# Jianxff/svo_pro_universal

Measured on AMD Instinct MI355X. Metric: aligned patches/sec + ms/frame, EuRoC 640x480 mono, 1/2/4/8 MI355X, higher is better.
Workload: dtype f64

## Files before the change

### svo_pro_universal_amd/csrc/context.hip

```cpp
#include <cmath>
#include <cstdarg>
#include <algorithm>
#include <cstring>

#include "svoh_internal.h"
#include "svoh_math.h"

namespace svoh {

static thread_local std::string g_global_err = "no error";

int set_error(svoh_ctx* ctx, int code, const char* fmt, ...)
{
  char buf[1024];
  va_list ap;
  va_start(ap, fmt);
  vsnprintf(buf, sizeof buf, fmt, ap);
  va_end(ap);
  if (ctx) ctx->err = buf; else g_global_err = buf;
  return code;
}

void set_global_error(const char* msg) { g_global_err = msg; }

// ... 351 lines not shown

__global__ __launch_bounds__(64) void camera_maths_wide_kernel(const svoh_camera cam, int n, const double* xyz, double* px, double* J, double* f_back)
{
  const int i = blockIdx.x * 64 + threadIdx.x;
  if (i >= n) return;
  const CamModelWide cm = load_camera_wide(cam);
  const Vec3 p = { xyz[3 * i], xyz[3 * i + 1], xyz[3 * i + 2] };
  double u, v;
  project3(cm, p, u, v);
  px[2 * i] = u; px[2 * i + 1] = v;
  if (J) {
    double Jl[6];
    project3_jacobian(cm, p, Jl);
    for (int k = 0; k < 6; ++k) J[6 * i + k] = Jl[k];
  }
  const Vec3 f = back_project3(cm, u, v);
  f_back[3 * i] = f.x; f_back[3 * i + 1] = f.y; f_back[3 * i + 2] = f.z;
}

void load_knobs_from_env(SvohKnobs& k)
{
  auto get = [](const char* name) { const char* e = getenv(name); return e ? atoi(e) : kKnobUnset; };
  k.klt_block = get("SVOH_KLT_BLOCK");
  k.matcher_g8 = get("SVOH_MATCHER_G8");
  k.seed_binning = get("SVOH_SEED_BINNING");
  k.pose_threads = get("SVOH_POSE_THREADS");
  k.align_cluster = get("SVOH_ALIGN_CLUSTER");
#ifdef SVOH_TEST_HOOKS
  k.align_cluster_test_absent = get("SVOH_ALIGN_CLUSTER_TEST_ABSENT");
#endif
  k.align_threads = get("SVOH_ALIGN_THREADS");
  k.align_rows = get("SVOH_ALIGN_ROWS");
  k.align_latency_build = get("SVOH_ALIGN_LATENCY_BUILD");
  k.align_lds = get("SVOH_ALIGN_LDS");
  k.align_wg_per_cu = get("SVOH_ALIGN_WG_PER_CU");
  k.kernel_timing = get("SVOH_KERNEL_TIMING");
  k.copy_kernel = get("SVOH_COPY_KERNEL");
}

static int build_pyramid_levels(svoh_ctx* ctx, hipStream_t stream, const std::shared_ptr<Slab>& slab, uint8_t* base, size_t fbytes, const size_t* offs, const int* ws,
                                const int* hs, int n_images, int width, int height, int n_levels, int rounding, svoh_frame_t* out_frames);

extern "C" {

int svoh_abi_version(void) { return SVOH_ABI_VERSION; }

int svoh_set_kernel_timing(svoh_ctx* ctx, int enabled)
try {
  if (!ctx) return set_error(nullptr, SVOH_ERR_INVALID_ARGUMENT, "ctx is NULL");
  ctx->knobs.kernel_timing = enabled ? 1 : 0;
  return SVOH_OK;
} SVOH_ABI_CATCH(ctx)

int svoh_set_copy_policy(svoh_ctx* ctx, int policy)
try {
  if (!ctx) return set_error(nullptr, SVOH_ERR_INVALID_ARGUMENT, "ctx is NULL");
  SVOH_REQUIRE(ctx, policy >= 0 && policy <= 2, "copy policy: 0 the runtime's copies, 1 copy kernels for 16 KB .. 1 MB, 2 copy kernels always");
  ctx->knobs.copy_kernel = policy;
  return SVOH_OK;
} SVOH_ABI_CATCH(ctx)

int svoh_reload_knobs(svoh_ctx* ctx)
try {
  if (!ctx) return set_error(nullptr, SVOH_ERR_INVALID_ARGUMENT, "ctx is NULL");
  const int timing = ctx->knobs.kernel_timing, copy_policy = ctx->knobs.copy_kernel;
  load_knobs_from_env(ctx->knobs);
// ... 465 lines not shown
```

### svo_pro_universal_amd/csrc/sparse_align.hip

```cpp
#include <atomic>
#include <cstdlib>
#include <cstring>

#include <type_traits>

#include "svoh_internal.h"
#include "svoh_device_utils.h"
#include "svoh_math.h"

#define SVOH_ALIGN_DRAIN(ctx) do { SVOH_HIP_TRY(ctx, hipStreamSynchronize((ctx)->stream)); (ctx)->align_launches_since_drain = 0; } while (0)

namespace svoh {

struct DevCamDesc {
  DevImage ref[SVOH_MAX_LEVELS];
  DevImage cur[SVOH_MAX_LEVELS];
  svoh_camera cam;
  svoh_se3 ref_T_imu_cam, ref_T_cam_imu, cur_T_cam_imu;
  double ref_pos[3];
  const double* px;
  const double* f;
  const double* pos_world;
  const uint8_t* flags;
  int32_t n_features;
// ... 6 lines not shown
  double alpha_init, beta_init;
  svoh_align_prior prior;
};

struct AlignKernelArgs {
  const DevProblemDesc* problems;
  const DevCamDesc* cams;
  svoh_align_result* results;
  double* wpk;
  int64_t slots;
  uint8_t* wsel;
  uint8_t* wvis;
  svoh_align_options opt;
  int32_t lds_img_bytes;
  int32_t rig_build;
  int32_t latency_build;
  int32_t lds_two_per_cu;
  int32_t ws_lds_bytes;
  int32_t eval_level;
  double* eval_out;
  long long* stamps;
  int32_t n_problems;
  int32_t* queue;
  int32_t one_each;
  const svoh_align_gn_state* ext_state;
  int32_t raw_sums;
  int32_t cluster;
  double* xchg;
  unsigned int* bar;
#ifdef SVOH_TEST_HOOKS
  int32_t cluster_test_absent;
#endif
};

constexpr int kXchgStride = 64;

#ifndef SVOH_ROW_UNROLL_GONLY
#define SVOH_ROW_UNROLL_GONLY 4
#endif
#ifndef SVOH_PIN_MOMENTS
#define SVOH_PIN_MOMENTS 1
#endif
#ifndef SVOH_ALIGN_WAVE_STEP
#define SVOH_ALIGN_WAVE_STEP 1
#endif
#ifndef SVOH_STEP_PRIO
#define SVOH_STEP_PRIO 1
#endif
#ifndef SVOH_ROW_UNROLL
#define SVOH_ROW_UNROLL (PH == 8 ? 4 : (D == 8 ? 1 : 2))
#endif

#ifdef SVOH_PHASE_STAMPS
#define SVOH_STAMP_DECL long long st_t0 = 0, st_acc[8] = {0, 0, 0, 0, 0, 0, 0, 0}; const long long st_begin = (long long)__builtin_amdgcn_s_memtime();
#define SVOH_STAMP_START() do { st_t0 = (long long)__builtin_amdgcn_s_memtime(); } while (0)
#define SVOH_STAMP_ADD(k) do { long long st_n = (long long)__builtin_amdgcn_s_memtime(); st_acc[k] += st_n - st_t0; st_t0 = st_n; } while (0)
#define SVOH_STAMP_COUNT(k) do { st_acc[k] += 1; } while (0)
#define SVOH_STAMP_FLUSH() do { if (threadIdx.x == 0) { st_acc[7] = (long long)__builtin_amdgcn_s_memtime() - st_begin; for (int k_ = 0; k_ < 8; ++k_) a.stamps[pbi * 20 + k_] = st_acc[k_]; for (int k_ = 0; k_ < 4; ++k_) a.stamps[pbi * 20 + 8 + k_] = g_state.dbg[k_]; for (int k_ = 0; k_ < 8; ++k_) a.stamps[pbi * 20 + 12 + k_] = g_state.dbg2[k_]; } } while (0)
#define SVOH_SERIAL_STAMP(k) do { long long st_n = (long long)__builtin_amdgcn_s_memtime(); s.dbg[k] += st_n - st_s0; st_s0 = st_n; } while (0)
#define SVOH_PASS_STAMP_BEGIN() long long ps_t0 = 0; if (threadIdx.x == 0) { __builtin_amdgcn_s_waitcnt(0); ps_t0 = (long long)__builtin_amdgcn_s_memtime(); }
#define SVOH_PASS_STAMP(k) do { if (threadIdx.x == 0) { __builtin_amdgcn_s_waitcnt(0); long long ps_n = (long long)__builtin_amdgcn_s_memtime(); g_state.dbg2[k] += ps_n - ps_t0; ps_t0 = ps_n; } } while (0)
#define SVOH_OUTER_STAMP_BEGIN() long long os_t0 = 0; if (threadIdx.x == 0) { __builtin_amdgcn_s_waitcnt(0); os_t0 = (long long)__builtin_amdgcn_s_memtime(); }
#define SVOH_OUTER_STAMP(k) do { if (threadIdx.x == 0) { __builtin_amdgcn_s_waitcnt(0); long long os_n = (long long)__builtin_amdgcn_s_memtime(); g_state.dbg2[k] += os_n - os_t0; os_t0 = os_n; } } while (0)
#else
#define SVOH_PASS_STAMP_BEGIN()
#define SVOH_PASS_STAMP(k) do {} while (0)
// ... 1066 lines not shown
    for (int j = 0; j < 8; ++j) { const double v = fabs(xg[j]); if (v > x_norm) x_norm = v; }
    if (x_norm < opt.eps) level_done = 1;
    __builtin_amdgcn_wave_barrier();
    if (lane == 0) {
      s.Told = T; s.alpha_old = alpha; s.beta_old = beta;
      s.T = Tn; s.alpha = an; s.beta = bn;
      if (level_done) s.level_done = 1;
    }
    T = Tn; alpha = an; beta = bn;
  }
  SVOH_WAVE_STAMP(2);
  {
    const int c = lane < n_cams ? lane : 0;
    const Rigid Tcr = mul(mul(s.cam_cur_T_cam_imu[c], T), s.cam_ref_T_imu_cam[c]);
    if (lane < n_cams) s.Tcr[c] = Tcr;
    if (lane == 0) { s.alpha_f = (float)alpha; s.beta_f = (float)beta; }
  }
  SVOH_WAVE_STAMP(3);
}

#ifndef SVOH_ALIGN_STAGED
#define SVOH_ALIGN_STAGED 1
#endif
#ifndef SVOH_ALIGN_REUSE_HESSIAN
#define SVOH_ALIGN_REUSE_HESSIAN 1
#endif
#ifndef SVOH_ALIGN_MIN_WAVES_256
#define SVOH_ALIGN_MIN_WAVES_256 2
#endif
#ifndef SVOH_ALIGN_ROWS_DEFAULT
#define SVOH_ALIGN_ROWS_DEFAULT(fit) (fit)
#endif

template <int P, int NT, bool ILLUM, bool CLUSTER = false, bool ROBUST = false, int LPP = 1, bool LAT = false, bool RIG = false>
__global__ __launch_bounds__(NT, (NT == 256 ? (LAT ? 1 : SVOH_ALIGN_MIN_WAVES_256) : 2))
void sparse_align_kernel(const AlignKernelArgs a)
{
  static_assert(!LAT || (NT == 256 && !CLUSTER && LPP == 1), "latency build: the 256-thread lane-per-patch geometry");
  static_assert(!RIG || (!CLUSTER && LPP == 1 && (LAT || NT == 512)), "rig build: the two lane-per-patch geometries of small launches");
  static_assert(LPP == 1 || (!CLUSTER && NT == 512 && LPP <= P), "rows geometry: 512 threads, no cluster mode");
  static_assert(NT == 256 || NT == 512, "workgroups of 256 or 512 threads");
  constexpr bool ROWS = LPP > 1;
  constexpr int D = ILLUM ? 8 : 6;
  constexpr int NACC = AccLayout<D>::NACC;
  constexpr int NW = NT / 64;

  constexpr bool STAGED = SVOH_ALIGN_STAGED && NT == 256 && !ROWS;
  constexpr bool kStageRegs = SVOH_ALIGN_STAGE_REGS != 0 && NT == 256 && !LAT && !CLUSTER && !ROWS;
  extern __shared__ __align__(16) unsigned char lds_img[];
  __shared__ __align__(16) double s_stage[STAGED ? NW * kStageDoubles : 2];
  __shared__ double s_jc[SVOH_MAX_CAMS][kJacConsts];
  __shared__ int s_lvl_off[SVOH_MAX_LEVELS];
  __shared__ double s_red[NW][NACC];
  static_assert(NACC <= 45, "g_sum is sized for the 8-parameter case");
  __shared__ double s_x[kXchgStride];
  __shared__ int s_cluster_ok;
  [[maybe_unused]] __shared__ __align__(16) LevelDesc s_lvd[SVOH_ALIGN_LDS_DESC ? SVOH_MAX_CAMS : 1];
  [[maybe_unused]] __shared__ int s_changed[SVOH_ALIGN_FOLD_VOTE ? NW : 1];

  const int tid = threadIdx.x;
  const int lane = tid & 63, wave = tid >> 6;
  __shared__ int s_pbi;
  __shared__ StageItem s_stage_items[kMaxStageItems];
#if SVOH_ALIGN_CLUSTER_XCD
  bool first_pull = true;
#endif
#if SVOH_ALIGN_ONE_EACH
  bool pulled_once = false;
#endif
  for (;;) {
// ... 79 lines not shown
              const int bytes = im.w * im.h;
              s_stage_items[n_items] = StageItem{ im.data, o, total16, bytes, 0 };
              ++n_items; total16 += bytes >> 4; o += (bytes + 15) & ~15;
            }
        } else {
          for (int c = 0; c < n_cams; ++c)
            for (int h = 0; h < 2; ++h) { const DevImage& im = h ? cams[c].cur[l] : cams[c].ref[l]; ++n_items; total16 += (im.w * im.h) >> 4; }
        }
        if (tid == 0) s_lvl_off[l] = off;
        off += need;
      }
      else if (tid == 0) s_lvl_off[l] = -1;
    }
    if (list_ok && n_items) {
      __syncthreads();
      stage_item_list<NT>(lds_img, s_stage_items, n_items, total16, tid);
    }
  }
#ifdef SVOH_STAGE_WAIT_EXPERIMENT
  __builtin_amdgcn_s_waitcnt(0x0F70);
  SVOH_STAMP_ADD(1);
#endif
  if (tid == 0) {
    g_state.T = load_rigid(pb.T_init);
    g_state.Told = g_state.T;
    g_state.alpha = pb.alpha_init; g_state.beta = pb.beta_init;
    if (a.ext_state) {
      g_state.T = load_rigid(a.ext_state->T_icur_iref);
      g_state.Told = g_state.T;
      g_state.alpha = a.ext_state->alpha; g_state.beta = a.ext_state->beta;
    }
    g_state.alpha_old = g_state.alpha; g_state.beta_old = g_state.beta;
    g_state.stop = 0; g_state.level_done = 0; g_state.nsel = 0; g_state.status = 0; g_state.patch_iters = 0;
    for (int k = 0; k < 8; ++k) g_state.I_prior[k] = 0.0;
    g_nvis = 0;
    g_state.prior = pb.prior;
    for (int c = 0; c < n_cams; ++c) {
      g_state.cam_cur_T_cam_imu[c] = load_rigid(cams[c].cur_T_cam_imu);
      g_state.cam_ref_T_imu_cam[c] = load_rigid(cams[c].ref_T_imu_cam);
      to_matrix(g_state.cam_ref_T_imu_cam[c].q, &s_jc[c][0]);
      s_jc[c][9] = g_state.cam_ref_T_imu_cam[c].t.x; s_jc[c][10] = g_state.cam_ref_T_imu_cam[c].t.y;
      s_jc[c][11] = g_state.cam_ref_T_imu_cam[c].t.z;
      to_matrix(load_rigid(cams[c].ref_T_cam_imu).q, &s_jc[c][12]);
    }
#ifdef SVOH_PHASE_STAMPS
    for (int k = 0; k < 4; ++k) g_state.dbg[k] = 0;
    for (int k = 0; k < 8; ++k) g_state.dbg2[k] = 0;
#endif
    for (int l = 0; l < SVOH_MAX_LEVELS; ++l) { g_state.lvl_iters[l] = 0; g_state.lvl_n_meas[l] = 0; g_state.lvl_chi2[l] = 0.0; }
  }
  __syncthreads();

  WsView ws = { a.wpk, a.slots, 0 };
  if constexpr (NT == 512) {
    if (a.ws_lds_bytes > 0) {
      int n_local = 0;
      for (int c = 0; c < n_cams; ++c) n_local += cams[c].n_features;
      if (n_local * kWsPairs * 16 <= a.ws_lds_bytes) {
        ws.base = reinterpret_cast<double*>(lds_img + a.lds_img_bytes);
        ws.slots = n_local;
        ws.first = cams[0].feat_off;
      }
    }
  }
  {
    int my_sel = 0;
    const int patch_size_wb = P + 2;
    const double scale = 1.0f / (1 << opt.max_level);
    const double patch_center_wb = (patch_size_wb - 1) / 2.0f;
    for (int c = 0; c < n_cams; ++c) {
      const DevCamDesc& cd = cams[c];
      const int rows_minus_two = cd.ref[opt.max_level].h - 2;
      const int cols_minus_two = cd.ref[opt.max_level].w - 2;
      struct FeatIn { double pu, pv, pwx, pwy, pwz, fx, fy, fz; unsigned flag; };
      auto request = [&](int k, FeatIn& o) {
        o.flag = cd.flags[k];
        o.pu = cd.px[2 * k]; o.pv = cd.px[2 * k + 1];
        o.pwx = cd.pos_world[3 * k + 0]; o.pwy = cd.pos_world[3 * k + 1]; o.pwz = cd.pos_world[3 * k + 2];
        o.fx = cd.f[3 * k + 0]; o.fy = cd.f[3 * k + 1]; o.fz = cd.f[3 * k + 2];
      };
#ifndef SVOH_ALIGN_BASE_DEPTH
#define SVOH_ALIGN_BASE_DEPTH 4
#endif
      constexpr int kBaseDepth = SVOH_ALIGN_BASE_DEPTH;
      for (int i0 = tid; i0 < cd.n_features; i0 += kBaseDepth * NT) {
        FeatIn in[kBaseDepth];
#pragma unroll
        for (int k = 0; k < kBaseDepth; ++k) {
          in[k] = FeatIn{ 0, 0, 0, 0, 0, 0, 0, 0, 0u };
          if (i0 + k * NT < cd.n_features) request(i0 + k * NT, in[k]);
        }
#pragma unroll
        for (int k = 0; k < kBaseDepth; ++k) {
          const int i = i0 + k * NT;
          if (i >= cd.n_features) break;
          const int gi = cd.feat_off + i;
          bool sel = in[k].flag != 0;
          const double pu = in[k].pu, pv = in[k].pv;
// ... 288 lines not shown
      if (eval_mode) { if (tid == 0) gn_serial_step<P, D, ILLUM>(a, pb, cams, n_cams, res_idx, level, iter, eval_mode, light); }
      else if (tid < 64) {
#if SVOH_STEP_PRIO
        __builtin_amdgcn_s_setprio(3);
#endif
        gn_wave_step<P, D, ILLUM>(a, n_cams, level, iter, light, tid);
#if SVOH_STEP_PRIO
        __builtin_amdgcn_s_setprio(0);
#endif
      }
#else
      if (tid == 0) gn_serial_step<P, D, ILLUM>(a, pb, cams, n_cams, res_idx, level, iter, eval_mode, light);
#endif
      __syncthreads();
      SVOH_STAMP_ADD(4);
      if (g_state.level_done) break;
    }
    if (cluster_failed) break;
  }

  if (tid == 0) {
    svoh_align_result& r = a.results[res_idx];
    r.status = cluster_failed ? 3 : g_state.status;
    r.n_fts_to_track = n_sel;
    store_rigid(g_state.T, r.T_icur_iref);
    r.alpha = g_state.alpha; r.beta = g_state.beta;
    r.n_patch_iters = g_state.patch_iters;
    for (int l = 0; l < SVOH_MAX_LEVELS; ++l) { r.iters[l] = g_state.lvl_iters[l]; r.n_meas[l] = g_state.lvl_n_meas[l]; r.chi2[l] = g_state.lvl_chi2[l]; }
  }
  SVOH_STAMP_FLUSH();
  }
}


__global__ __launch_bounds__(128)
void sum_shares_kernel(const double* parts, int n_shares, double* out)
{
  const int k = threadIdx.x;
  if (k >= 74) return;
  double v = 0.0;
  for (int s = 0; s < n_shares; ++s) v += parts[74 * s + k];
  out[k] = v;
}

template <int P, bool ILLUM>
__global__ __launch_bounds__(64)
void align_gn_update_kernel(const AlignKernelArgs a, const double* sums, svoh_align_gn_state* st, int level, int iter)
{
  constexpr int D = ILLUM ? 8 : 6;
  constexpr int NH = AccLayout<D>::NH;
  ShState& s = g_state;
  double (&s_sum)[45] = g_sum;
  if (threadIdx.x != 0) return;
  const DevProblemDesc& pb = a.problems[0];
  const DevCamDesc* cams = a.cams + pb.cam_begin;
  s.T = load_rigid(st->T_icur_iref);
  s.alpha = st->alpha; s.beta = st->beta;
  if (iter == 0) {
    s.Told = s.T; s.alpha_old = s.alpha; s.beta_old = s.beta;
    for (int k = 0; k < 8; ++k) s.I_prior[k] = 0.0;
  } else {
    s.Told = load_rigid(st->T_old); s.alpha_old = st->alpha_old; s.beta_old = st->beta_old;
    for (int k = 0; k < 8; ++k) s.I_prior[k] = st->I_prior[k];
  }
  s.stop = st->stop; s.status = st->status; s.level_done = 0; s.nsel = 0; s.patch_iters = 0;
  {
    int idx = 0;
    for (int r = 0; r < D; ++r)
      for (int c2 = r; c2 < D; ++c2) s_sum[idx++] = sums[c2 * 8 + r];
    for (int r = 0; r < D; ++r) s_sum[NH + r] = sums[64 + r];
    s_sum[NH + D] = sums[72];
  }
  const int n_meas = (int)sums[73];
  g_nvis = n_meas / (P * P);
  s.prior = pb.prior;
  for (int c = 0; c < pb.n_cams; ++c) {
    s.cam_cur_T_cam_imu[c] = load_rigid(cams[c].cur_T_cam_imu);
    s.cam_ref_T_imu_cam[c] = load_rigid(cams[c].ref_T_imu_cam);
  }
  gn_serial_step<P, D, ILLUM>(a, pb, cams, pb.n_cams, 0, level, iter, false, false);
  if (level < SVOH_MAX_LEVELS) {
    svoh_align_result& res = a.results[0];
    res.iters[level] = s.lvl_iters[level]; res.n_meas[level] = s.lvl_n_meas[level]; res.chi2[level] = s.lvl_chi2[level];
  }
  store_rigid(s.T, st->T_icur_iref);
  st->alpha = s.alpha; st->beta = s.beta;
  store_rigid(s.Told, st->T_old);
  st->alpha_old = s.alpha_old; st->beta_old = s.beta_old;
  for (int k = 0; k < 8; ++k) st->I_prior[k] = s.I_prior[k];
  st->chi2 = s_sum[NH + D] / (double)n_meas;
  st->n_meas = n_meas;
  st->stop = s.stop; st->level_done = s.level_done; st->status = s.status;
}

struct LaunchCfg { int nt; size_t lds; };

constexpr size_t kLdsPerCu = 163840;
template <int P, int NT, bool ILLUM, bool CLUSTER, bool ROBUST, int LPP = 1, bool LAT = false, bool RIG = false>
static hipError_t launch_one(hipStream_t st, int grid, size_t lds, AlignKernelArgs args)
{
  auto kern = sparse_align_kernel<P, NT, ILLUM, CLUSTER, ROBUST, LPP, LAT, RIG>;
  if (NT == 256 && args.lds_two_per_cu) {
    static std::atomic<size_t> static_lds_cache{ 0 };
    size_t static_lds = static_lds_cache.load(std::memory_order_relaxed);
    if (static_lds == 0) {
      hipFuncAttributes attr;
      hipError_t ea = hipFuncGetAttributes(&attr, reinterpret_cast<const void*>(kern));
      if (ea != hipSuccess) return ea;
      static_lds = attr.sharedSizeBytes ? attr.sharedSizeBytes : 1;
      static_lds_cache.store(static_lds, std::memory_order_relaxed);
    }
    const size_t room = kLdsPerCu / 2 > static_lds ? (kLdsPerCu / 2 - static_lds) & ~(size_t)15 : 0;
    if (lds > room) {
      args.lds_img_bytes -= (int32_t)(lds - room);
      if (args.lds_img_bytes < 0) args.lds_img_bytes = 0;
      lds = room;
    }
  }
  hipError_t e = hipFuncSetAttribute(reinterpret_cast<const void*>(kern),
                                     hipFuncAttributeMaxDynamicSharedMemorySize, (int)lds);
  if (e != hipSuccess) return e;
  hipLaunchKernelGGL(kern, dim3(grid), dim3(NT), lds, st, args);
  return hipGetLastError();
}

template <int P, bool ILLUM, bool ROBUST>
static hipError_t launch_nt(hipStream_t st, int nt, int lpp, int grid, size_t lds, const AlignKernelArgs& args)
{
  if (args.cluster > 1) return launch_one<P, 256, ILLUM, true, ROBUST>(st, grid, lds, args);
  if (nt == 256) {
    if (args.latency_build) return args.rig_build ? launch_one<P, 256, ILLUM, false, ROBUST, 1, true, true>(st, grid, lds, args)
                                                  : launch_one<P, 256, ILLUM, false, ROBUST, 1, true>(st, grid, lds, args);
    return launch_one<P, 256, ILLUM, false, ROBUST>(st, grid, lds, args);
  }
  if (lpp <= 1 && args.rig_build) return launch_one<P, 512, ILLUM, false, ROBUST, 1, false, true>(st, grid, lds, args);
  switch (lpp) {
    case 2: return launch_one<P, 512, ILLUM, false, ROBUST, 2>(st, grid, lds, args);
    case 4: return launch_one<P, 512, ILLUM, false, ROBUST, 4>(st, grid, lds, args);
    case 8: if constexpr (P == 8) return launch_one<P, 512, ILLUM, false, ROBUST, 8>(st, grid, lds, args);
    default: return launch_one<P, 512, ILLUM, false, ROBUST>(st, grid, lds, args);
  }
}

constexpr int kWsLdsMaxFeatures = 340;
constexpr int kClusterMinFeatures = 512;
constexpr int kClusterMaxWorkgroups = 32;
constexpr int kClusterMaxProblems = 64;

static int validate_options(svoh_ctx* ctx, const svoh_align_options* o)
{
  SVOH_REQUIRE(ctx, o != nullptr, "options is NULL");
  if (o->patch_size != 4 && o->patch_size != 8)
    return set_error(ctx, SVOH_ERR_UNSUPPORTED, "patch_size %d not built (4 and 8 are)", o->patch_size);
  SVOH_REQUIRE(ctx, o->max_level >= o->min_level && o->min_level >= 0 && o->max_level < SVOH_MAX_LEVELS,
               "bad level range");
  SVOH_REQUIRE(ctx, o->max_iter >= 1, "max_iter must be >= 1");
  return SVOH_OK;
}

struct SplitArgs {
  const svoh_align_gn_state* ext_state = nullptr;
  double* sums_out = nullptr;
  const double* sums_in = nullptr;
  svoh_align_gn_state* state = nullptr;
  int iter = 0;
  bool update = false;
  int n_shares = 1;
};

struct AlignGeometry {
  int cluster_g = 0;
  int nt = 256;
  int rows = 1;
  bool latency = false;
  bool rig = false;
  int32_t key() const { return (1 << 30) | (cluster_g & 0xff) | ((nt == 512 ? 1 : 0) << 8) | ((rows & 0xf) << 9) | ((latency ? 1 : 0) << 13) | ((rig ? 1 : 0) << 14); }
  static bool from_key(int32_t k, AlignGeometry* g)
  {
    if (!(k & (1 << 30)) || (k & ~((1 << 30) | 0x7fff))) return false;
    g->cluster_g = k & 0xff; g->nt = (k >> 8) & 1 ? 512 : 256; g->rows = (k >> 9) & 0xf; g->latency = (k >> 13) & 1; g->rig = (k >> 14) & 1;
    return (g->rows == 1 || g->rows == 2 || g->rows == 4 || g->rows == 8) && g->cluster_g != 1 && g->cluster_g <= kClusterMaxWorkgroups;
  }
};

static int decide_cluster(const svoh_ctx* ctx, int n_problems, const svoh_align_problem* problems)
{
  if (n_problems > kClusterMaxProblems || ctx->align_no_cluster) return 0;
  int64_t nf_min = INT64_MAX, nf_max = 0;
  for (int p = 0; p < n_problems; ++p) {
    int64_t nf = 0;
    if (problems[p].n_cams >= 1 && problems[p].n_cams <= SVOH_MAX_CAMS)
      for (int c = 0; c < problems[p].n_cams; ++c) nf += problems[p].cams[c].n_features > 0 ? problems[p].cams[c].n_features : 0;
    nf_min = nf < nf_min ? nf : nf_min;
    nf_max = nf > nf_max ? nf : nf_max;
  }
  int g = SvohKnobs::or_default(ctx->knobs.align_cluster, -1);
  const bool worth = nf_min >= kClusterMinFeatures && (n_problems <= 16 || nf_min >= 3000);
  auto workgroups_for = [](int64_t nf) {
    if (nf < 875) return 3;
    if (nf < 1250) return 4;
    if (nf < 1750) return 6;
    if (nf < 5000) return 8;
    if (nf < 7000) return 12;
    if (nf < 16000) return 16;
    return 20;
  };
  if (g < 0) g = worth ? workgroups_for(nf_max) : 0;
  if (g > kClusterMaxWorkgroups) g = kClusterMaxWorkgroups;
  if ((int64_t)g * n_problems > ctx->num_cus) g = ctx->num_cus / n_problems;
  return g >= 2 ? g : 0;
}

struct LaunchShape { int max_feat_per_problem = 0; bool have_rig = false, rig_wants_512 = false; };
static void add_to_shape(const svoh_align_problem& pb, int S, LaunchShape* z)
{
  int nf = 0;
// ... 134 lines not shown
    if (need > ctx->d_results.cap) {
      if (dev_results_off) {
        SVOH_ALIGN_DRAIN(ctx);
        DevBuffer bigger;
        SVOH_HIP_TRY(ctx, bigger.reserve(need * 2));
        SVOH_HIP_TRY(ctx, hipMemcpy(bigger.ptr, ctx->d_results.ptr, sizeof(svoh_align_result) * dev_results_off, hipMemcpyDeviceToDevice));
        std::swap(bigger.ptr, ctx->d_results.ptr);
        std::swap(bigger.cap, ctx->d_results.cap);
      } else {
        SVOH_HIP_TRY(ctx, ctx->d_results.reserve(need));
      }
    }
  }
  if (delivers) {
    SVOH_REQUIRE(ctx, ctx->align_pending_results + (size_t)n_problems <= svoh_ctx::kMaxQueuedResults,
                 "too many alignment results queued without a fetch");
    size_t want_results = ctx->align_pending_results + (size_t)n_problems;
    const size_t queue_of_these = (size_t)svoh_ctx::kAlignEventRing * (size_t)n_problems;
    if (want_results < queue_of_these && queue_of_these <= svoh_ctx::kMaxQueuedResults) want_results = queue_of_these;
    const size_t need = sizeof(svoh_align_result) * want_results;
    if (need > ctx->h_results.cap) {
      if (ctx->align_pending_results) {
        SVOH_ALIGN_DRAIN(ctx);
        PinnedBuffer bigger;
        SVOH_HIP_TRY(ctx, bigger.reserve(need * 2));
        memcpy(bigger.ptr, ctx->h_results.ptr, sizeof(svoh_align_result) * ctx->align_pending_results);
        std::swap(bigger.ptr, ctx->h_results.ptr);
        std::swap(bigger.cap, ctx->h_results.cap);
      } else {
        SVOH_HIP_TRY(ctx, ctx->h_results.reserve(need));
      }
    }
  }
  SVOH_HIP_TRY(ctx, ctx->d_feat.reserve(feat_slots * (kWsPairs * 16 + 2) + 256));
  SVOH_HIP_TRY(ctx, ctx->d_eval.reserve(74 * sizeof(double) * S));

  DevProblemDesc* hp = static_cast<DevProblemDesc*>(h_desc.ptr);
  DevCamDesc* hc = reinterpret_cast<DevCamDesc*>(hp + n_desc);
  uint8_t* hup = static_cast<uint8_t*>(h_desc.ptr) + up_base;
  uint8_t* dup = static_cast<uint8_t*>(ctx->d_desc.ptr) + up_base;
  size_t up_off = 0;
  int cam_idx = 0, feat_off = 0;
  const int need_levels = opt->max_level + 1;
  const uint8_t* share_base[SVOH_MAX_CAMS] = {};
  std::vector<PosFromSeedsJob> pos_jobs;
  int pos_jobs_max_n = 0;
  for (int pd = 0; pd < n_desc; ++pd) {
    const int p = pd / S, sh = pd % S;
    const svoh_align_problem& pb = problems[p];
    DevProblemDesc& d = hp[pd];
    d.n_cams = pb.n_cams;
    d.cam_begin = cam_idx;
    d.T_init = pb.T_icur_iref;
    d.alpha_init = pb.alpha_init; d.beta_init = pb.beta_init;
    d.prior = pb.prior;
    for (int c = 0; c < pb.n_cams; ++c, ++cam_idx) {
      const svoh_align_camera& cam = pb.cams[c];
      DevCamDesc& dc = hc[cam_idx];
      const Frame* fr = find_frame(ctx, cam.ref_frame);
      const Frame* fc = find_frame(ctx, cam.cur_frame);
      if (!fr || !fc) return set_error(ctx, SVOH_ERR_BAD_HANDLE, "problem %d camera %d: unknown frame handle", p, c);
      if (fr->n_levels < need_levels || fc->n_levels < need_levels)
        return set_error(ctx, SVOH_ERR_INVALID_ARGUMENT, "problem %d camera %d: pyramid has fewer than %d levels", p,
                         c, need_levels);
      for (int l = 0; l < SVOH_MAX_LEVELS; ++l) {
        dc.ref[l] = l < fr->n_levels ? fr->lv[l] : DevImage{ nullptr, 0, 0, 0, 0 };
        dc.cur[l] = l < fc->n_levels ? fc->lv[l] : DevImage{ nullptr, 0, 0, 0, 0 };
// ... 115 lines not shown
  args.queue = reinterpret_cast<int32_t*>(static_cast<uint8_t*>(ctx->d_desc.ptr) + ctl_off);
#ifdef SVOH_PHASE_STAMPS
  SVOH_HIP_TRY(ctx, ctx->d_scratch0.reserve(sizeof(long long) * 20 * (size_t)n_problems));
  args.stamps = static_cast<long long*>(ctx->d_scratch0.ptr);
#endif

  const AlignGeometry geo = forced ? *forced : decide_geometry(ctx, opt, n_desc, cluster ? S : 0, shape);
  const int nt = geo.nt, rows = geo.rows;
  size_t lds = (nt == 256) ? 52224 : 78 * 1024;
  args.latency_build = geo.latency ? 1 : 0;
  args.rig_build = geo.rig ? 1 : 0;
  args.lds_two_per_cu = (nt == 256 && !cluster && ctx->knobs.align_lds == kKnobUnset && ctx->knobs.align_wg_per_cu == kKnobUnset) ? 1 : 0;
  lds = (size_t)SvohKnobs::or_default(ctx->knobs.align_lds, (int)lds) & ~(size_t)15;
  const size_t lds_cap = (nt == 256 && SVOH_ALIGN_STAGED) ? 163840 - 32768 : 153856;
  if (lds > lds_cap) lds = lds_cap;
  args.ws_lds_bytes = 0;
  if (nt == 512 && !cluster && max_feat_per_problem <= kWsLdsMaxFeatures && lds >= (size_t)kWsLdsMaxFeatures * kWsPairs * 16 + 4096) {
    args.ws_lds_bytes = ((max_feat_per_problem > 0 ? max_feat_per_problem : 1) * kWsPairs * 16 + 15) & ~15;
  }
  args.lds_img_bytes = (int32_t)(lds - (size_t)args.ws_lds_bytes);

  const bool illum = opt->estimate_illumination_gain || opt->estimate_illumination_offset;
  int grid = ctx->num_cus * SvohKnobs::or_default(ctx->knobs.align_wg_per_cu, nt == 256 ? 2 : 1);
  if (grid > n_desc || grid <= 0) grid = n_desc;
  if (cluster) grid = n_desc;
  args.one_each = (!cluster && grid == n_desc) ? 1 : 0;
#if SVOH_ALIGN_CLUSTER_XCD
  if (cluster) grid = 8 * args.cluster * ((n_desc / args.cluster + 7) / 8);
#endif
  hipError_t e;
  const bool timed = ctx->timing_on();
  const int ev_slot = (int)(ctx->align_timed_launches % svoh_ctx::kAlignEventRing);
  if (timed) SVOH_HIP_TRY(ctx, hipEventRecord(ctx->ev_align_start[ev_slot], ctx->stream));
  const bool robust = opt->robustification != 0;
#ifdef SVOH_DEV_ONLY_PLAIN
  if (robust || illum) return set_error(ctx, SVOH_ERR_UNSUPPORTED, "development build: plain kernels only");
  e = opt->patch_size == 4 ? launch_nt<4, false, false>(ctx->stream, nt, rows, grid, lds, args)
                           : launch_nt<8, false, false>(ctx->stream, nt, rows, grid, lds, args);
#else
  if (opt->patch_size == 4) {
    if (robust) e = illum ? launch_nt<4, true, true>(ctx->stream, nt, rows, grid, lds, args) : launch_nt<4, false, true>(ctx->stream, nt, rows, grid, lds, args);
    else e = illum ? launch_nt<4, true, false>(ctx->stream, nt, rows, grid, lds, args) : launch_nt<4, false, false>(ctx->stream, nt, rows, grid, lds, args);
  } else {
    if (robust) e = illum ? launch_nt<8, true, true>(ctx->stream, nt, rows, grid, lds, args) : launch_nt<8, false, true>(ctx->stream, nt, rows, grid, lds, args);
    else e = illum ? launch_nt<8, true, false>(ctx->stream, nt, rows, grid, lds, args) : launch_nt<8, false, false>(ctx->stream, nt, rows, grid, lds, args);
  }
#endif
  if (e != hipSuccess)
    return set_error(ctx, SVOH_ERR_HIP, "sparse_align launch failed: %s", hipGetErrorString(e));
  if (S > 1 && !cluster) {
    hipLaunchKernelGGL(sum_shares_kernel, dim3(1), dim3(128), 0, ctx->stream, static_cast<const double*>(ctx->d_eval.ptr), S,
                       split->sums_out);
    const hipError_t es = hipGetLastError();
    if (es != hipSuccess) return set_error(ctx, SVOH_ERR_HIP, "sum_shares launch failed: %s", hipGetErrorString(es));
  }
  if (timed) { SVOH_HIP_TRY(ctx, hipEventRecord(ctx->ev_align_stop[ev_slot], ctx->stream)); ++ctx->align_timed_launches; }
  ctx->align_last_timed = timed;
  ++ctx->align_launches;
  if (!split && eval_level < 0) {
    ctx->align_last_geometry_key = geo.key(); ctx->align_last_grid = grid; ctx->align_last_n_desc = n_desc;
  }
  if (delivers) {
    SVOH_HIP_TRY(ctx, svoh_copy_to_host(ctx, static_cast<svoh_align_result*>(ctx->h_results.ptr) + ctx->align_pending_results,
                                        args.results, sizeof(svoh_align_result) * n_problems));
    ctx->align_last_results_off = ctx->align_pending_results;
    if (ctx->align_pending_results == 0) ctx->align_result_dev_index.clear();
    for (int p = 0; p < n_problems; ++p) ctx->align_result_dev_index.push_back((uint32_t)(dev_results_off + (size_t)p));
    ctx->align_pending_results += (size_t)n_problems;
    ctx->align_pending_dev = dev_results_off + (size_t)n_desc + (size_t)n_problems;
  }
#ifdef SVOH_PHASE_STAMPS
  {
    std::vector<long long> h((size_t)n_problems * 20);
    SVOH_HIP_TRY(ctx, hipMemcpyAsync(h.data(), args.stamps, h.size() * sizeof(long long), hipMemcpyDeviceToHost, ctx->stream));
    SVOH_ALIGN_DRAIN(ctx);
    double sum[20] = {0};
    for (int p = 0; p < n_problems; ++p) for (int k = 0; k < 20; ++k) sum[k] += (double)h[(size_t)p * 20 + k];
    fprintf(stderr, "[stamps] one-lane step: set-up %.0f solve %.0f update %.0f camera poses %.0f\n", sum[8] / n_problems, sum[9] / n_problems,
            sum[10] / n_problems, sum[11] / n_problems);
    fprintf(stderr, "[stamps] inside the passes (thread 0): set-up %.0f row arrival %.0f projection %.0f pixels %.0f Jacobian rows + map %.0f; gradient-only passes as a whole %.0f, the vote's barrier behind them %.0f\n", sum[12] / n_problems,
            sum[13] / n_problems, sum[14] / n_problems, sum[15] / n_problems, sum[16] / n_problems, sum[17] / n_problems, sum[18] / n_problems);
    fprintf(stderr, "[stamps] n=%d nt=%d avg cycles/block: base %.0f stage %.0f patch %.0f reduce %.0f serial %.0f total %.0f; "
            "gradient-only passes kept %.2f / discarded %.2f per problem\n",
            n_problems, nt, sum[0] / n_problems, sum[1] / n_problems, sum[2] / n_problems, sum[3] / n_problems,
            sum[4] / n_problems, sum[7] / n_problems, sum[6] / n_problems, sum[5] / n_problems);
  }
#endif
  ctx->last_align_n = delivers ? n_problems : 0;
  return SVOH_OK;
}

}

// ... 235 lines not shown
```

### svo_pro_universal_amd/csrc/svoh_internal.h

```cpp
#pragma once

#include <hip/hip_runtime.h>

#include <cstdint>
#include <cstdio>
#include <memory>
#include <new>
#include <stdexcept>
#include <string>
#include <unordered_map>
#include <algorithm>
#include <vector>

#include "../../include/svo_hip.h"

namespace svoh {

struct DevImage {
  const uint8_t* data;
  int32_t w, h, pitch, pad;
};

constexpr size_t kSlabTailPad = 64;

// ... 110 lines not shown
};

struct PinnedBuffer {
  void* ptr = nullptr;
  size_t cap = 0;
  hipError_t reserve(size_t bytes)
  {
    if (bytes <= cap) return hipSuccess;
    if (ptr) { (void)hipHostFree(ptr); ptr = nullptr; cap = 0; }
    size_t want = bytes + bytes / 2 + 4096;
    if (want < kMinScratchBytes) want = kMinScratchBytes;
    hipError_t e = hipHostMalloc(&ptr, want, hipHostMallocDefault);
    if (e == hipSuccess) cap = want;
    return e;
  }
  ~PinnedBuffer() { if (ptr) (void)hipHostFree(ptr); }
};

}

constexpr int kKnobUnset = -2147483647 - 1;
struct SvohKnobs {
  int klt_block = kKnobUnset;
  int matcher_g8 = kKnobUnset;
  int seed_binning = kKnobUnset;
  int pose_threads = kKnobUnset;
  int align_cluster = kKnobUnset;
#ifdef SVOH_TEST_HOOKS
  int align_cluster_test_absent = kKnobUnset;
#endif
  int align_threads = kKnobUnset;
  int align_rows = kKnobUnset;
  int align_latency_build = kKnobUnset;
  int align_lds = kKnobUnset;
  int align_wg_per_cu = kKnobUnset;
  int kernel_timing = kKnobUnset;
  int copy_kernel = kKnobUnset;
  static int or_default(int v, int dflt) { return v == kKnobUnset ? dflt : v; }
};
void load_knobs_from_env(SvohKnobs& k);

struct svoh_ctx {
  SvohKnobs knobs;
  int device = 0;
  hipStream_t stream = nullptr;
  int num_cus = 0;
  size_t lds_per_block = 0;
  std::string err;
  std::shared_ptr<svoh::SlabPool> slab_pool = std::make_shared<svoh::SlabPool>();
  std::unordered_map<uint64_t, svoh::Frame> frames;
  uint64_t next_frame_id = 1;
  uint64_t handle_generation = 0;
  std::shared_ptr<svoh::BlockPool> feature_pool = std::make_shared<svoh::BlockPool>();
  std::unordered_map<uint64_t, svoh::FeatureSet> feature_sets;
  uint64_t next_features_id = 1;
  svoh::PinnedBuffer h_features;
  hipEvent_t ev_features = nullptr;

  svoh::DevBuffer d_desc;
  svoh::DevBuffer d_results;
  svoh::DevBuffer d_feat;
  svoh::DevBuffer d_eval;
  svoh::DevBuffer d_xchg;
  svoh::DevBuffer d_split;
  svoh::PinnedBuffer h_desc;
  svoh::PinnedBuffer h_desc_odd;
// ... 138 lines not shown
```

### svo_pro_universal_amd/frontend.py

```python
import ctypes as C

import numpy as np

from . import _capi as capi


class SvohError(RuntimeError):
    def __init__(self, code, msg):
        RuntimeError.__init__(self, "svoh error %d: %s" % (code, msg))
        self.code = code


def _se3(T):
    s = capi.svoh_se3()
    v = T.as7() if hasattr(T, "as7") else np.asarray(T, dtype=np.float64)
    for i in range(4):
        s.q[i] = float(v[i])
    for i in range(3):
        s.t[i] = float(v[4 + i])
    return s


def _camera(cam):
    c = capi.svoh_camera()
# ... 112 lines not shown
        w, h = C.c_int(), C.c_int()
        self._check(self.lib.svoh_download_level(self.h, frame, level, None, C.byref(w), C.byref(h)))
        out = np.zeros((h.value, w.value), dtype=np.uint8)
        self._check(self.lib.svoh_download_level(self.h, frame, level, out.ctypes.data, C.byref(w), C.byref(h)))
        return out

    def release_frame(self, frame):
        self._check(self.lib.svoh_release_frame(self.h, frame))

    def sparse_align(self, opt, problems):
        n = len(problems)
        res = (capi.svoh_align_result * n)()
        self._check(self.lib.svoh_sparse_align_batch(self.h, C.byref(opt), n, problems, res))
        return res

    def sparse_align_enqueue(self, opt, problems):
        self._check(self.lib.svoh_sparse_align_enqueue(self.h, C.byref(opt), len(problems), problems))

    def sparse_align_fetch(self, n):
        res = (capi.svoh_align_result * n)()
        self._check(self.lib.svoh_sparse_align_fetch(self.h, n, res))
        return res

    def sparse_align_fetch_all(self, n_total):
        res = (capi.svoh_align_result * n_total)()
        self._check(self.lib.svoh_sparse_align_fetch_all(self.h, n_total, res))
        return res

    def last_align_launch(self):
        key, grid, n_desc = C.c_int32(), C.c_int32(), C.c_int32()
        self._check(self.lib.svoh_sparse_align_last_launch_info(self.h, C.byref(key), C.byref(grid), C.byref(n_desc)))
        k = key.value
        return dict(key=k, cluster_g=k & 0xff, nt=512 if (k >> 8) & 1 else 256, rows=(k >> 9) & 0xf,
                    latency=bool((k >> 13) & 1), rig=bool((k >> 14) & 1), grid=grid.value, n_desc=n_desc.value)

    def sparse_align_evaluate(self, opt, problem, level):
        H = np.zeros(64)
        g = np.zeros(8)
        chi2, nm, nsel = C.c_double(), C.c_int32(), C.c_int32()
        ntot = sum(problem.cams[i].n_features for i in range(problem.n_cams))
        vis = np.zeros(max(1, ntot), np.uint8)
        self._check(self.lib.svoh_sparse_align_evaluate(self.h, C.byref(opt), C.byref(problem), level,
                                                        H.ctypes.data, g.ctypes.data, C.byref(chi2), C.byref(nm),
                                                        vis.ctypes.data, C.byref(nsel)))
        return H.reshape(8, 8).T.copy(), g, chi2.value, nm.value, vis[:nsel.value].copy()

    def split_init(self, problem, d_state):
        self._check(self.lib.svoh_sparse_align_split_init(self.h, C.byref(problem), C.c_void_p(d_state)))

    def partial_sums(self, opt, problem, level, d_state, d_sums, n_workgroups=0):
        self._check(self.lib.svoh_sparse_align_partial_sums(self.h, C.byref(opt), C.byref(problem), level,
                                                            n_workgroups, C.c_void_p(d_state), C.c_void_p(d_sums)))

    def gn_update(self, opt, problem, level, it, d_sums, d_state):
        st = capi.svoh_align_gn_state()
        self._check(self.lib.svoh_sparse_align_gn_update(self.h, C.byref(opt), C.byref(problem), level, it,
                                                         C.c_void_p(d_sums), C.c_void_p(d_state), C.byref(st)))
        return st


def fill_align_camera(cam_struct, scene, ref_frame, cur_frame, keep, device_ptrs=None):
    cam_struct.ref_frame = ref_frame
    cam_struct.cur_frame = cur_frame
    cam_struct.cam = _camera(scene.cam)
    cam_struct.ref_T_imu_cam = _se3(scene.T_imu_cam)
    cam_struct.ref_T_cam_imu = _se3(scene.T_cam_imu)
    cam_struct.cur_T_cam_imu = _se3(scene.T_cam_imu)
# ... 249 lines not shown
```

Before: 2.132 billion.

## Move sparse-align per-feature base setup into a separate pre-pass kernel

Adds an align_base_kernel launched with one workgroup per camera. It does the per-feature selection, back-projection to 3D and workspace writes, and counts selected features per camera. The main 256-thread batch kernel gets a PREBASE template variant that skips its own setup block and sums the precomputed counts instead. The goal is to take the serial setup work out of the main alignment kernel, so it is spread across more workgroups and the main kernel starts iterating sooner. In exchange there is an extra kernel launch per align call and another kernel template instantiation. The path is on by default and can be turned off with the SVOH_ALIGN_PREPASS environment variable.

```diff
diff --git a/svo_pro_universal_amd/csrc/context.hip b/svo_pro_universal_amd/csrc/context.hip
--- a/svo_pro_universal_amd/csrc/context.hip
+++ b/svo_pro_universal_amd/csrc/context.hip
@@ -407,6 +407,7 @@
   k.align_threads = get("SVOH_ALIGN_THREADS");
   k.align_rows = get("SVOH_ALIGN_ROWS");
   k.align_latency_build = get("SVOH_ALIGN_LATENCY_BUILD");
+  k.align_prepass = get("SVOH_ALIGN_PREPASS");
   k.align_lds = get("SVOH_ALIGN_LDS");
   k.align_wg_per_cu = get("SVOH_ALIGN_WG_PER_CU");
   k.kernel_timing = get("SVOH_KERNEL_TIMING");
diff --git a/svo_pro_universal_amd/csrc/sparse_align.hip b/svo_pro_universal_amd/csrc/sparse_align.hip
--- a/svo_pro_universal_amd/csrc/sparse_align.hip
+++ b/svo_pro_universal_amd/csrc/sparse_align.hip
@@ -62,6 +62,10 @@
   int32_t cluster_test_absent;
 #endif
 };
+struct AlignKernelArgsPre : AlignKernelArgs {
+  const int32_t* cam_nsel;
+};
+constexpr int kLppPrebase = 0;
 
 constexpr int kXchgStride = 64;
 
@@ -1194,10 +1198,13 @@
 #define SVOH_ALIGN_ROWS_DEFAULT(fit) (fit)
 #endif
 
-template <int P, int NT, bool ILLUM, bool CLUSTER = false, bool ROBUST = false, int LPP = 1, bool LAT = false, bool RIG = false>
+template <int P, int NT, bool ILLUM, bool CLUSTER = false, bool ROBUST = false, int LPP_ = 1, bool LAT = false, bool RIG = false>
 __global__ __launch_bounds__(NT, (NT == 256 ? (LAT ? 1 : SVOH_ALIGN_MIN_WAVES_256) : 2))
-void sparse_align_kernel(const AlignKernelArgs a)
-{
+void sparse_align_kernel(const std::conditional_t<LPP_ == kLppPrebase, AlignKernelArgsPre, AlignKernelArgs> a)
+{
+  constexpr bool PREBASE = LPP_ == kLppPrebase;
+  constexpr int LPP = PREBASE ? 1 : LPP_;
+  static_assert(!PREBASE || (NT == 256 && !LAT && !CLUSTER && !RIG), "pre-pass: the batch build only");
   static_assert(!LAT || (NT == 256 && !CLUSTER && LPP == 1), "latency build: the 256-thread lane-per-patch geometry");
   static_assert(!RIG || (!CLUSTER && LPP == 1 && (LAT || NT == 512)), "rig build: the two lane-per-patch geometries of small launches");
   static_assert(LPP == 1 || (!CLUSTER && NT == 512 && LPP <= P), "rows geometry: 512 threads, no cluster mode");
@@ -1343,6 +1350,8 @@
     }
     g_state.alpha_old = g_state.alpha; g_state.beta_old = g_state.beta;
     g_state.stop = 0; g_state.level_done = 0; g_state.nsel = 0; g_state.status = 0; g_state.patch_iters = 0;
+    if constexpr (PREBASE)
+      for (int c = 0; c < n_cams; ++c) g_state.nsel += a.cam_nsel[pb.cam_begin + c];
     for (int k = 0; k < 8; ++k) g_state.I_prior[k] = 0.0;
     g_nvis = 0;
     g_state.prior = pb.prior;
@@ -1374,7 +1383,7 @@
       }
     }
   }
-  {
+  if constexpr (!PREBASE) {
     int my_sel = 0;
     const int patch_size_wb = P + 2;
     const double scale = 1.0f / (1 << opt.max_level);
@@ -1729,6 +1738,68 @@
   }
 }
 
+constexpr int kBaseThreads = 256;
+__global__ __launch_bounds__(kBaseThreads)
+void align_base_kernel(const DevCamDesc* __restrict__ cams, int max_level, int patch_size, double* __restrict__ wpk, int64_t slots,
+                       uint8_t* __restrict__ wsel, uint8_t* __restrict__ wvis, int32_t* __restrict__ cam_nsel)
+{
+  __shared__ int s_cnt[kBaseThreads / 64];
+  const int tid = threadIdx.x;
+  const DevCamDesc& cd = cams[blockIdx.x];
+  const WsView ws = { wpk, slots, 0 };
+  const int patch_size_wb = patch_size + 2;
+  const double scale = 1.0f / (1 << max_level);
+  const double patch_center_wb = (patch_size_wb - 1) / 2.0f;
+  const int rows_minus_two = cd.ref[max_level].h - 2;
+  const int cols_minus_two = cd.ref[max_level].w - 2;
+  const int n = cd.n_features;
+  const int feat_off = cd.feat_off;
+  const uint8_t* __restrict__ flags = cd.flags;
+  const double* __restrict__ px = cd.px;
+  const double* __restrict__ pos_world = cd.pos_world;
+  const double* __restrict__ f = cd.f;
+  const double rpx = cd.ref_pos[0], rpy = cd.ref_pos[1], rpz = cd.ref_pos[2];
+  int my_sel = 0;
+  for (int i = tid; i < n; i += kBaseThreads) {
+    const int gi = feat_off + i;
+    bool sel = flags[i] != 0;
+    const double pu = px[2 * i], pv = px[2 * i + 1];
+    const double pwx = pos_world[3 * i + 0], pwy = pos_world[3 * i + 1], pwz = pos_world[3 * i + 2];
+    const double fx_ = f[3 * i + 0], fy_ = f[3 * i + 1], fz_ = f[3 * i + 2];
+    if (sel) {
+      const double u_tl = pu * scale - patch_center_wb;
+      const double v_tl = pv * scale - patch_center_wb;
+      const int u_tl_i = (int)floor(u_tl);
+      const int v_tl_i = (int)floor(v_tl);
+      sel = !(u_tl_i < 0 || v_tl_i < 0 || u_tl_i >= cols_minus_two - patch_size_wb ||
+              v_tl_i >= rows_minus_two - patch_size_wb);
+    }
+    wsel[gi] = sel ? 1 : 0;
+    wvis[gi] = 0;
+    if (!sel) *reinterpret_cast<double2*>(ws_pair(ws, 2, gi)) = make_double2(0.0, 0.0);
+    if (sel) {
+      const double dx = pwx - rpx;
+      const double dy = pwy - rpy;
+      const double dz = pwz - rpz;
+      const double depth = sqrt(dx * dx + dy * dy + dz * dz);
+      const Vec3 X = { fx_ * depth, fy_ * depth, fz_ * depth };
+      *reinterpret_cast<double2*>(ws_pair(ws, 0, gi)) = make_double2(X.x, X.y);
+      *reinterpret_cast<double2*>(ws_pair(ws, 1, gi)) = make_double2(X.z, pu);
+      *reinterpret_cast<double2*>(ws_pair(ws, 2, gi)) = make_double2(pv, 1.0);
+      ++my_sel;
+    }
+  }
+#pragma unroll
+  for (int o = 32; o >= 1; o >>= 1) my_sel += __shfl_xor(my_sel, o);
+  if ((tid & 63) == 0) s_cnt[tid >> 6] = my_sel;
+  __syncthreads();
+  if (tid == 0) {
+    int total = 0;
+    for (int w = 0; w < kBaseThreads / 64; ++w) total += s_cnt[w];
+    cam_nsel[blockIdx.x] = total;
+  }
+}
+
 
 __global__ __launch_bounds__(128)
 void sum_shares_kernel(const double* parts, int n_shares, double* out)
@@ -1794,7 +1865,7 @@
 
 constexpr size_t kLdsPerCu = 163840;
 template <int P, int NT, bool ILLUM, bool CLUSTER, bool ROBUST, int LPP = 1, bool LAT = false, bool RIG = false>
-static hipError_t launch_one(hipStream_t st, int grid, size_t lds, AlignKernelArgs args)
+static hipError_t launch_one(hipStream_t st, int grid, size_t lds, std::conditional_t<LPP == kLppPrebase, AlignKernelArgsPre, AlignKernelArgs> args)
 {
   auto kern = sparse_align_kernel<P, NT, ILLUM, CLUSTER, ROBUST, LPP, LAT, RIG>;
   if (NT == 256 && args.lds_two_per_cu) {
@@ -1822,12 +1893,18 @@
 }
 
 template <int P, bool ILLUM, bool ROBUST>
-static hipError_t launch_nt(hipStream_t st, int nt, int lpp, int grid, size_t lds, const AlignKernelArgs& args)
+static hipError_t launch_nt(hipStream_t st, int nt, int lpp, int grid, size_t lds, const AlignKernelArgs& args, const int32_t* cam_nsel)
 {
   if (args.cluster > 1) return launch_one<P, 256, ILLUM, true, ROBUST>(st, grid, lds, args);
   if (nt == 256) {
     if (args.latency_build) return args.rig_build ? launch_one<P, 256, ILLUM, false, ROBUST, 1, true, true>(st, grid, lds, args)
                                                   : launch_one<P, 256, ILLUM, false, ROBUST, 1, true>(st, grid, lds, args);
+    if (cam_nsel) {
+      AlignKernelArgsPre pre;
+      static_cast<AlignKernelArgs&>(pre) = args;
+      pre.cam_nsel = cam_nsel;
+      return launch_one<P, 256, ILLUM, false, ROBUST, kLppPrebase>(st, grid, lds, pre);
+    }
     return launch_one<P, 256, ILLUM, false, ROBUST>(st, grid, lds, args);
   }
   if (lpp <= 1 && args.rig_build) return launch_one<P, 512, ILLUM, false, ROBUST, 1, false, true>(st, grid, lds, args);
@@ -1879,6 +1956,8 @@
     return (g->rows == 1 || g->rows == 2 || g->rows == 4 || g->rows == 8) && g->cluster_g != 1 && g->cluster_g <= kClusterMaxWorkgroups;
   }
 };
+
+constexpr int32_t kLaunchInfoPrepassBit = 1 << 15;
 
 static int decide_cluster(const svoh_ctx* ctx, int n_problems, const svoh_align_problem* problems)
 {
@@ -2079,7 +2158,8 @@
       }
     }
   }
-  SVOH_HIP_TRY(ctx, ctx->d_feat.reserve(feat_slots * (kWsPairs * 16 + 2) + 256));
+  const size_t cam_nsel_off = (feat_slots * (kWsPairs * 16 + 2) + 256 + 3) & ~(size_t)3;
+  SVOH_HIP_TRY(ctx, ctx->d_feat.reserve(cam_nsel_off + sizeof(int32_t) * n_cams_total));
   SVOH_HIP_TRY(ctx, ctx->d_eval.reserve(74 * sizeof(double) * S));
 
   DevProblemDesc* hp = static_cast<DevProblemDesc*>(h_desc.ptr);
@@ -2261,18 +2341,28 @@
   const bool timed = ctx->timing_on();
   const int ev_slot = (int)(ctx->align_timed_launches % svoh_ctx::kAlignEventRing);
   if (timed) SVOH_HIP_TRY(ctx, hipEventRecord(ctx->ev_align_start[ev_slot], ctx->stream));
+  const bool prepass = nt == 256 && !geo.latency && !cluster && !split && eval_level < 0 &&
+                       SvohKnobs::or_default(ctx->knobs.align_prepass, 1) != 0;
+  int32_t* cam_nsel = nullptr;
+  if (prepass) {
+    cam_nsel = reinterpret_cast<int32_t*>(static_cast<uint8_t*>(ctx->d_feat.ptr) + cam_nsel_off);
+    hipLaunchKernelGGL(align_base_kernel, dim3((unsigned)n_cams_total), dim3(kBaseThreads), 0, ctx->stream, args.cams, (int)opt->max_level,
+                       (int)opt->patch_size, args.wpk, args.slots, args.wsel, args.wvis, cam_nsel);
+    const hipError_t eb = hipGetLastError();
+    if (eb != hipSuccess) return set_error(ctx, SVOH_ERR_HIP, "align_base launch failed: %s", hipGetErrorString(eb));
+  }
   const bool robust = opt->robustification != 0;
 #ifdef SVOH_DEV_ONLY_PLAIN
   if (robust || illum) return set_error(ctx, SVOH_ERR_UNSUPPORTED, "development build: plain kernels only");
-  e = opt->patch_size == 4 ? launch_nt<4, false, false>(ctx->stream, nt, rows, grid, lds, args)
-                           : launch_nt<8, false, false>(ctx->stream, nt, rows, grid, lds, args);
+  e = opt->patch_size == 4 ? launch_nt<4, false, false>(ctx->stream, nt, rows, grid, lds, args, cam_nsel)
+                           : launch_nt<8, false, false>(ctx->stream, nt, rows, grid, lds, args, cam_nsel);
 #else
   if (opt->patch_size == 4) {
-    if (robust) e = illum ? launch_nt<4, true, true>(ctx->stream, nt, rows, grid, lds, args) : launch_nt<4, false, true>(ctx->stream, nt, rows, grid, lds, args);
-    else e = illum ? launch_nt<4, true, false>(ctx->stream, nt, rows, grid, lds, args) : launch_nt<4, false, false>(ctx->stream, nt, rows, grid, lds, args);
+    if (robust) e = illum ? launch_nt<4, true, true>(ctx->stream, nt, rows, grid, lds, args, cam_nsel) : launch_nt<4, false, true>(ctx->stream, nt, rows, grid, lds, args, cam_nsel);
+    else e = illum ? launch_nt<4, true, false>(ctx->stream, nt, rows, grid, lds, args, cam_nsel) : launch_nt<4, false, false>(ctx->stream, nt, rows, grid, lds, args, cam_nsel);
   } else {
-    if (robust) e = illum ? launch_nt<8, true, true>(ctx->stream, nt, rows, grid, lds, args) : launch_nt<8, false, true>(ctx->stream, nt, rows, grid, lds, args);
-    else e = illum ? launch_nt<8, true, false>(ctx->stream, nt, rows, grid, lds, args) : launch_nt<8, false, false>(ctx->stream, nt, rows, grid, lds, args);
+    if (robust) e = illum ? launch_nt<8, true, true>(ctx->stream, nt, rows, grid, lds, args, cam_nsel) : launch_nt<8, false, true>(ctx->stream, nt, rows, grid, lds, args, cam_nsel);
+    else e = illum ? launch_nt<8, true, false>(ctx->stream, nt, rows, grid, lds, args, cam_nsel) : launch_nt<8, false, false>(ctx->stream, nt, rows, grid, lds, args, cam_nsel);
   }
 #endif
   if (e != hipSuccess)
@@ -2287,7 +2377,7 @@
   ctx->align_last_timed = timed;
   ++ctx->align_launches;
   if (!split && eval_level < 0) {
-    ctx->align_last_geometry_key = geo.key(); ctx->align_last_grid = grid; ctx->align_last_n_desc = n_desc;
+    ctx->align_last_geometry_key = geo.key() | (prepass ? kLaunchInfoPrepassBit : 0); ctx->align_last_grid = grid; ctx->align_last_n_desc = n_desc;
   }
   if (delivers) {
     SVOH_HIP_TRY(ctx, svoh_copy_to_host(ctx, static_cast<svoh_align_result*>(ctx->h_results.ptr) + ctx->align_pending_results,
diff --git a/svo_pro_universal_amd/csrc/svoh_internal.h b/svo_pro_universal_amd/csrc/svoh_internal.h
--- a/svo_pro_universal_amd/csrc/svoh_internal.h
+++ b/svo_pro_universal_amd/csrc/svoh_internal.h
@@ -166,6 +166,7 @@
   int align_threads = kKnobUnset;
   int align_rows = kKnobUnset;
   int align_latency_build = kKnobUnset;
+  int align_prepass = kKnobUnset;
   int align_lds = kKnobUnset;
   int align_wg_per_cu = kKnobUnset;
   int kernel_timing = kKnobUnset;
diff --git a/svo_pro_universal_amd/frontend.py b/svo_pro_universal_amd/frontend.py
--- a/svo_pro_universal_amd/frontend.py
+++ b/svo_pro_universal_amd/frontend.py
@@ -168,7 +168,7 @@
         self._check(self.lib.svoh_sparse_align_last_launch_info(self.h, C.byref(key), C.byref(grid), C.byref(n_desc)))
         k = key.value
         return dict(key=k, cluster_g=k & 0xff, nt=512 if (k >> 8) & 1 else 256, rows=(k >> 9) & 0xf,
-                    latency=bool((k >> 13) & 1), rig=bool((k >> 14) & 1), grid=grid.value, n_desc=n_desc.value)
+                    latency=bool((k >> 13) & 1), rig=bool((k >> 14) & 1), prepass=bool((k >> 15) & 1), grid=grid.value, n_desc=n_desc.value)
 
     def sparse_align_evaluate(self, opt, problem, level):
         H = np.zeros(64)
```

Result: no change. 2.130 billion (-0.1%).
